# torognes/swarm

Hardware: AMD Instinct MI355X
Metric: amplicons/sec clustered (d=1) (higher is better)
Workload: dtype u64; 1 GPU; 10000000 synthetic amplicons x 150 bp, d=1 (10000000 per GPU; the metric's own size; configs[1]: configs1); per_gpu_queries=10000000, db_amplicons=10000000, step=swa_d1_index_build + swa_d1_network_device (B1 seam), db and CSR resident in HBM, route=streaming (d1_stream.inc), build=local, neighbour_links=17077441

## Files before the change

### swarm_amd/csrc/d1.hip

```cpp
#include "swa_internal.h"

#include <algorithm>
#include <type_traits>
#include <cstdlib>
#include <memory>
#include <thread>

namespace {

constexpr int kWaves = 4;
constexpr int kThreads = kWaves * 64;
constexpr int kQueueCap = 128;
constexpr size_t kMaxZobristLds = SWA_MAX_ZOBRIST_LDS;

#include "wave_ops.inc"
#include "group_join.inc"

struct alignas(16) swa_task {
  uint64_t hash;
  uint32_t heavy;
  uint32_t code;
};

struct NetArgs {
// ... 717 lines not shown
static int launch_abundance_rank(swa_ctx * ctx) {
  if (ctx->up.d1.rank_ready) {
    if (ctx->up.d1.db_unordered) { SWA_HIP(ctx, hipMemsetAsync(swa_status(ctx)->flags + kFlagUnordered, 1, sizeof(uint32_t), ctx->stream)); }
    return SWA_OK;
  }
  ctx->up.d1.rank_ready = true;
  SWA_HIP(ctx, hipMemsetAsync(swa_status(ctx)->flags + kFlagUnordered, 0, sizeof(uint32_t), ctx->stream));
  const uint32_t n = ctx->db.n;
  const uint32_t tiles = (n + 255u) / 256u;
  SWA_TRY(swa_reserve(ctx, ctx->d_arank, uint64_t(n) * sizeof(uint32_t)));
  SWA_TRY(swa_reserve(ctx, ctx->d_rank_tmp, uint64_t(tiles) * sizeof(uint32_t)));
  auto * rank = static_cast<uint32_t *>(ctx->d_arank.ptr);
  auto * tile_last = static_cast<uint32_t *>(ctx->d_rank_tmp.ptr);
  hipLaunchKernelGGL(k_abundance_rank, dim3(grid_for(ctx, n, 256, 8)), dim3(256), 0, ctx->stream, ctx->db.abundance, n, rank,
                     swa_status(ctx)->flags, tile_last);
  hipLaunchKernelGGL(k_abundance_rank_carry, dim3(1), dim3(256), 0, ctx->stream, tile_last, tiles);
  hipLaunchKernelGGL(k_abundance_rank_fill, dim3(grid_for(ctx, n, 256, 8)), dim3(256), 0, ctx->stream, n, rank, tile_last);
  return SWA_OK;
}

__global__ void k_set_flags(uint32_t * flags, uint32_t unserved, uint32_t shortest_code) { flags[kFlagUnserved] = unserved; flags[kFlagShortest] = shortest_code; }
__global__ void k_set_guard_made(unsigned long long * guard, uint32_t made0, uint32_t made1) { guard[kGuardMade] = made0; guard[kGuardMade + 1] = made1; }


using PartPlan = swa_part_levels;

struct PartJob {
  uint32_t nidx = 1;
  const unsigned long long * in[kMaxIdx] = {};
  unsigned long long * buf[kMaxIdx][2] = {};
  const uint64_t * cstart0[kMaxIdx] = {};
  uint64_t cstride0[kMaxIdx] = {};
  const uint32_t * csize0[kMaxIdx] = {};
  uint32_t csize_cap = 0, chunks0 = 1;
  bool single0 = true;
  uint64_t max_records = 0, max_tiles0 = 0;
  uint64_t out_cap = 0;
  uint32_t bias = 0, top_bit = 32;
  uint32_t tile = 4096;
  bool hist0_done = false;
  bool tiles0_done = false;
  const SegArgs * seg = nullptr;
  PartPlan plan{};
  uint32_t * cnt[kMaxIdx] = {}; uint32_t * ctile[kMaxIdx] = {}; uint64_t * starts[kMaxIdx] = {}; uint32_t * partial[kMaxIdx] = {};
  uint32_t * total[kMaxIdx] = {};
  uint64_t starts_stride = 0;
  const unsigned long long * out[kMaxIdx] = {}; const uint64_t * bstart[kMaxIdx] = {};
  uint32_t buckets = 0;
  int last = 0;
};

static void part_scratch(const PartJob & j, uint64_t * cnt, uint64_t * ctile, uint64_t * starts_half, uint64_t * partial) {
  uint64_t chunks = j.chunks0, c_max = 0, t_max = 0, s_max = 0;
  bool single = j.single0;
  for (uint32_t l = 0; l < j.plan.levels; ++l) {
    const uint64_t tiles = (l == 0 ? j.max_tiles0 : j.max_records / j.tile + chunks + 1);
    c_max = std::max(c_max, (tiles << j.plan.bits[l]) + 2);
    t_max = std::max(t_max, chunks + 2 + tiles + 2);
    chunks = (single ? 1 : chunks) << j.plan.bits[l];
    single = false;
    s_max = std::max(s_max, chunks + 2);
  }
  *cnt = c_max; *ctile = t_max; *starts_half = s_max; *partial = c_max / kFlatChunk + 2;
}

struct ClearList { uint32_t * p[8]; uint64_t words[8]; uint32_t n; };
__global__ __launch_bounds__(256) void k_clear_many(const ClearList c) {
  for (uint32_t k = 0; k < c.n; ++k) {
    for (uint64_t i = (uint64_t)blockIdx.x * blockDim.x + threadIdx.x; i < c.words[k]; i += (uint64_t)gridDim.x * blockDim.x) { c.p[k][i] = 0u; }
  }
}
static void clear_add(ClearList & c, void * p, uint64_t bytes) {
  c.p[c.n] = static_cast<uint32_t *>(p); c.words[c.n] = bytes / 4; ++c.n;
}
static int clear_launch(swa_ctx * ctx, const ClearList & c) {
  uint64_t most = 0;
  for (uint32_t k = 0; k < c.n; ++k) { most = std::max(most, c.words[k]); }
  if (c.n == 0 || most == 0) { return SWA_OK; }
  hipLaunchKernelGGL(k_clear_many, dim3(grid_for(ctx, most, 256, 8)), dim3(256), 0, ctx->stream, c);
  SWA_HIP(ctx, hipGetLastError());
  return SWA_OK;
}

static int run_partition(swa_ctx * ctx, PartJob & j) {
  uint64_t chunks = j.chunks0;
  bool single = j.single0;
  uint32_t used_bits = 0;
  const int cu_grid = ctx->num_cus * 8;
  for (uint32_t l = 0; l < j.plan.levels; ++l) {
    const uint32_t bits = j.plan.bits[l];
    used_bits += bits;
    const bool wide = bits > kPartMaxBits;
    const bool hist_done = l == 0 && j.hist0_done;
    const bool have_form = wide ? j.tile == 4096 || (j.tile == 8192 && hist_done) : j.tile == 2048 || j.tile == 4096;
    if (!have_form) { return swa_fail_msg(ctx, SWA_E_ARG, "partition: no kernel for this tile and bin count"); }
    PartArgs a{};
    a.single_seg = single ? 1u : 0u; a.bits = bits; a.shift = j.top_bit - used_bits; a.bias = j.bias; a.tile = j.tile;
    a.span = (single && l == 0 && chunks > 1 && j.tile == 4096 && !wide && !hist_done) ? 1u : 0u;
    const uint64_t tiles = (l == 0 ? j.max_tiles0 : j.max_records / j.tile + chunks + 1);
    a.run_bits = tiles >= (uint64_t)cu_grid ? 4u : 0u;
    for (uint32_t i = 0; i < j.nidx; ++i) {
      PartIdx & p = a.p[i];
      p.in = l == 0 ? j.in[i] : j.buf[i][(l - 1) & 1u];
      p.out = j.buf[i][l & 1u];
      p.out_cap = j.out_cap;
      p.cstart = l == 0 ? j.cstart0[i] : j.starts[i] + ((l - 1) & 1u) * j.starts_stride;
      p.cstride = l == 0 ? j.cstride0[i] : 0;
      p.csize = l == 0 ? j.csize0[i] : nullptr;
      p.csize_cap = j.csize_cap;
      p.chunks = (uint32_t)chunks;
      p.ctile = j.ctile[i]; p.cnt = j.cnt[i];
      p.tchunk = j.ctile[i] + chunks + 1; p.tchunk_cap = (uint32_t)std::min<uint64_t>(tiles + 1, 0xFFFFFFFFu);
      p.next_start = j.starts[i] + (l & 1u) * j.starts_stride;
      p.total = j.total[i];
    }
    const dim3 grid_t((unsigned)((std::min<uint64_t>(std::max<uint64_t>(tiles, 1), (uint64_t)cu_grid) + 7) & ~7ull), j.nidx);
    if (hist_done && j.tiles0_done) {  }
    else if (l == 0 && j.seg != nullptr) {
      if (chunks > 2048) { hipLaunchKernelGGL((k_part_tiles<1024, true>), dim3(1, 1), dim3(1024), 0, ctx->stream, a, *j.seg); }
      else { hipLaunchKernelGGL((k_part_tiles<256, true>), dim3(1, 1), dim3(256), 0, ctx->stream, a, *j.seg); }
    }
    else if (chunks > 2048) { hipLaunchKernelGGL(k_part_tiles<1024>, dim3(1, j.nidx), dim3(1024), 0, ctx->stream, a, SegArgs{}); }
    else { hipLaunchKernelGGL(k_part_tiles<256>, dim3(1, j.nidx), dim3(256), 0, ctx->stream, a, SegArgs{}); }
    if (hist_done) {  }
    else if (wide) { hipLaunchKernelGGL((k_part_hist<1024, kPartTileMax, 256>), grid_t, dim3(256), 0, ctx->stream, a); }
    else if (a.span != 0u) { hipLaunchKernelGGL((k_part_hist<512, kPartTileMax, 256, true>), grid_t, dim3(256), 0, ctx->stream, a); }
    else { hipLaunchKernelGGL((k_part_hist<512, kPartTileMax, 256>), grid_t, dim3(256), 0, ctx->stream, a); }
    FlatScanArgs f{};
    f.unit_bits = bits;
    for (uint32_t i = 0; i < j.nidx; ++i) { f.v[i] = j.cnt[i]; f.units[i] = j.ctile[i] + chunks; f.partial[i] = j.partial[i]; f.total[i] = j.total[i]; }
    const dim3 grid_f((unsigned)std::min<uint64_t>(((tiles << bits) + 1 + kFlatChunk - 1) / kFlatChunk, (uint64_t)cu_grid), j.nidx);
    hipLaunchKernelGGL(k_flat_sums, grid_f, dim3(256), 0, ctx->stream, f);
    hipLaunchKernelGGL(k_flat_apply, grid_f, dim3(256), 0, ctx->stream, f);
    if (wide && j.tile == 8192) {
      constexpr size_t lds = part_scatter_lds(8192, 1024);
      if (!ctx->part_lds_opt_in) {
        SWA_HIP(ctx, hipFuncSetAttribute(reinterpret_cast<const void *>(&k_part_scatter<8192, 1024, 1024>), hipFuncAttributeMaxDynamicSharedMemorySize, (int)lds));
        ctx->part_lds_opt_in = true;
      }
      hipLaunchKernelGGL((k_part_scatter<8192, 1024, 1024>), grid_t, dim3(1024), lds, ctx->stream, a);
    }
    else if (wide) { hipLaunchKernelGGL((k_part_scatter<4096, 1024, 512>), grid_t, dim3(512), part_scatter_lds(4096, 1024), ctx->stream, a); }
    else if (j.tile == 2048) { hipLaunchKernelGGL((k_part_scatter<2048, 512, 512>), grid_t, dim3(512), part_scatter_lds(2048, 512), ctx->stream, a); }
    else if (a.span != 0u) { hipLaunchKernelGGL((k_part_scatter<4096, 512, 512, true>), grid_t, dim3(512), part_scatter_lds(4096, 512), ctx->stream, a); }
    else { hipLaunchKernelGGL((k_part_scatter<4096, 512, 512>), grid_t, dim3(512), part_scatter_lds(4096, 512), ctx->stream, a); }
    chunks = (single ? 1 : chunks) << bits;
    single = false;
    SWA_HIP(ctx, hipGetLastError());
  }
  j.buckets = (uint32_t)chunks;
  j.last = (int)((j.plan.levels - 1) & 1u);
  for (uint32_t i = 0; i < j.nidx; ++i) {
    j.out[i] = j.buf[i][j.last];
    j.bstart[i] = j.starts[i] + (uint64_t)j.last * j.starts_stride;
  }
  return SWA_OK;
}

static int ensure_lines(swa_ctx * ctx) {
  const uint32_t lq = line_quads_for(ctx);
  if (ctx->up.d1.lines_ready && ctx->up.d1.lines_quads == lq) { return SWA_OK; }
  const uint32_t n = ctx->db.n;
  SWA_TRY(swa_reserve(ctx, ctx->d_stream[kSbLines], (uint64_t)n * lq * 16u + 64u));
  auto * lines = static_cast<uint4 *>(ctx->d_stream[kSbLines].ptr);
  const auto * rank = static_cast<const uint32_t *>(ctx->d_arank.ptr);
  SWA_HIP(ctx, hipMemsetAsync(reinterpret_cast<uint8_t *>(lines) + (uint64_t)n * lq * 16u, 0, 64, ctx->stream));
  swa_t0(ctx, kTimeLines);
  const dim3 grid(grid_for(ctx, n, 256, 8));
  if (lq == 4u) { hipLaunchKernelGGL(k_lines_build<4>, grid, dim3(256), 0, ctx->stream, ctx->db.seqs, ctx->db.seq_off, ctx->db.seqlen, rank, n, lines); }
  else if (lq == 8u) { hipLaunchKernelGGL(k_lines_build<8>, grid, dim3(256), 0, ctx->stream, ctx->db.seqs, ctx->db.seq_off, ctx->db.seqlen, rank, n, lines); }
  else { hipLaunchKernelGGL(k_lines_build<16>, grid, dim3(256), 0, ctx->stream, ctx->db.seqs, ctx->db.seq_off, ctx->db.seqlen, rank, n, lines); }
  swa_t1(ctx, kTimeLines);
  SWA_HIP(ctx, hipGetLastError());
  ctx->up.d1.lines_ready = true;
  ctx->up.d1.lines_quads = lq;
  return SWA_OK;
}

struct RouteLists {
  const uint32_t * ids[2] = {nullptr, nullptr};
  const unsigned long long * rec[2] = {nullptr, nullptr};
  uint32_t m[2] = {0, 0};
  bool routed() const { return ids[0] != nullptr || rec[0] != nullptr; }
  bool by_rec() const { return rec[0] != nullptr; }
};

static int build_stream_index(swa_ctx * ctx, const RouteLists & route) {
  const bool clear_head = ctx->ix.head_clear_pending;
  ctx->ix.head_clear_pending = false;
  ctx->ix.anchor_ready = false;
  ctx->ix.stream_index = false;
  ctx->ix.list_counts_ready = false;
  const uint32_t n = ctx->db.n;
  swa_status_block * st = swa_status(ctx);
  swa_lap(ctx, "(build starts)");
  SWA_TRY(ensure_db_lengths(ctx));
  swa_lap(ctx, "db lengths");
  SWA_TRY(ensure_lines(ctx));
  swa_lap(ctx, "amplicon lines");
  const uint32_t lq = ctx->up.d1.lines_quads;
  uint64_t item_room = 0;
  const ListRegions regions = list_regions(ctx, &item_room);
  const bool by_rec = route.by_rec();
  const bool routed = route.routed();
  const uint64_t records = routed ? std::max<uint64_t>(std::max(route.m[0], route.m[1]), 1) : n;
  uint32_t forced_bits = 0;
  if (const char * e = getenv("SWA_D1_PART_BITS")) {
    const int b = atoi(e);
    if (b >= 1 && b <= (int)(3 * kPartMaxBits)) { forced_bits = (uint32_t)b; }
  }
  const swa_part_plan plan = swa_part_plan_for(records, ctx->up.d1.stream_extra_bits, routed, forced_bits);
  const uint32_t total_bits = plan.lv.total;
  const bool keys_hist = plan.keys_hist;
  PartJob j;
  j.nidx = 2;
  j.plan = plan.lv;
  j.max_records = records;
  j.out_cap = records + 1;
  j.tile = plan.tile;
  swa_part_plan_report(plan, ctx->ix.part_plan);
  ctx->ix.part_plan[7] = ctx->up.d1.stream_extra_bits;
  ctx->ix.part_starts_valid = false;
  j.max_tiles0 = records / j.tile + 2;
// ... 59 lines not shown
    hipLaunchKernelGGL(k_set_flags, dim3(1), dim3(1), 0, ctx->stream, dflags,
                       ctx->up.d1.db_shortest < minlen ? 1u : 0u, 0xFFFFFFFFu - ctx->up.d1.db_shortest);
  }
  if (by_rec) {
    hipLaunchKernelGGL(k_set_guard_made, dim3(1), dim3(1), 0, ctx->stream, k.guard, route.m[0], route.m[1]);
  }
  swa_t0(ctx, kTimeKeys);
  if (by_rec) {  }
  else if (keys_hist) {
    const uint32_t ntiles = (uint32_t)((records + j.tile - 1) / j.tile);
    for (int i = 0; i < 2; ++i) {
      k.hist_cnt[i] = static_cast<uint32_t *>(ctx->d_stream[kSbCnt + i].ptr);
      k.hist_ctile[i] = static_cast<uint32_t *>(ctx->d_stream[kSbTile + i].ptr);
    }
    k.hist_bits = j.plan.bits[0]; k.hist_tile = j.tile; k.hist_ntiles = ntiles;
    k.hist_run_bits = j.max_tiles0 >= (uint64_t)ctx->num_cus * 8 ? 4u : 0u;
    const dim3 hgrid((unsigned)((std::min<uint64_t>(ntiles, (uint64_t)ctx->num_cus * 8) + 7) & ~7ull), 1u);
    hipLaunchKernelGGL(k_keys<true>, hgrid, dim3(256), 0, ctx->stream, k);
    j.hist0_done = true;
    j.tiles0_done = true;
  } else {
    const dim3 kgrid((unsigned)grid_for(ctx, records, 256, 8), routed ? 2u : 1u);
    hipLaunchKernelGGL(k_keys<false>, kgrid, dim3(256), 0, ctx->stream, k);
  }
  swa_t1(ctx, kTimeKeys);
  swa_lap(ctx, "k_keys");

  for (int i = 0; i < 2; ++i) {
    j.buf[i][0] = static_cast<unsigned long long *>(ctx->d_stream[kSbRec + 2 * i].ptr);
    j.buf[i][1] = static_cast<unsigned long long *>(ctx->d_stream[kSbRec + 2 * i + 1].ptr);
    j.in[i] = by_rec ? route.rec[i] : j.buf[i][1];
    j.cstart0[i] = nullptr; j.cstride0[i] = routed ? route.m[i] : n;
    j.cnt[i] = static_cast<uint32_t *>(ctx->d_stream[kSbCnt + i].ptr);
    j.ctile[i] = static_cast<uint32_t *>(ctx->d_stream[kSbTile + i].ptr);
    j.starts[i] = static_cast<uint64_t *>(ctx->d_stream[kSbStart + i].ptr);
    j.partial[i] = static_cast<uint32_t *>(ctx->d_stream[kSbPartial + i].ptr);
    j.total[i] = reinterpret_cast<uint32_t *>(scal + 8 + i);
  }
  j.starts_stride = e_start + 2;
  swa_t0(ctx, kTimeKeyPartition);
  SWA_TRY(run_partition(ctx, j));
  swa_t1(ctx, kTimeKeyPartition);
  swa_lap(ctx, "key partition");
  ctx->ix.part_starts_at = (uint64_t)(j.bstart[0] - j.starts[0]);
  ctx->ix.part_buckets = j.buckets;
  ctx->ix.part_starts_valid = true;
  if (!ctx->up.d1.guard_keys_done) {
    auto * guard = reinterpret_cast<unsigned long long *>(st->guard);
    SWA_HIP(ctx, hipMemsetAsync(guard + kGuardKeys, 0, sizeof(st->guard) - kGuardKeys * sizeof(uint64_t), ctx->stream));
    GuardDbArgs gd{};
    gd.seqs = ctx->db.seqs; gd.seq_off = ctx->db.seq_off; gd.seqlen = ctx->db.seqlen; gd.n = n;
    for (int i = 0; i < 2; ++i) { gd.list[i] = k.list[i]; gd.list_count[i] = routed ? route.m[i] : 0; gd.list_rec[i] = by_rec ? route.rec[i] : nullptr; }
    gd.owner_rank = k.owner_rank; gd.owner_world = k.owner_world; gd.win_a = win_a; gd.win_b = win_b; gd.nwin = k.nwin;
    gd.out = guard + kGuardKeysDb;
    hipLaunchKernelGGL(k_guard_db, dim3((unsigned)grid_for(ctx, records, 256, 8), routed ? 2u : 1u), dim3(256), 0, ctx->stream, gd);
    GuardRecArgs gr{};
    for (int i = 0; i < 2; ++i) { gr.rec[i] = j.out[i]; gr.total[i] = j.total[i]; }
    gr.out = guard + kGuardKeysRec;
    hipLaunchKernelGGL(k_guard_records, dim3((unsigned)grid_for(ctx, records, 256, 8), 2u), dim3(256), 0, ctx->stream, gr);
    ctx->up.d1.guard_keys_pending = true;
  }

  swa_lap(ctx, "guard: second opinion");
  GroupArgs g{};
  for (int i = 0; i < 2; ++i) {
    GroupIdx & x = g.g[i];
    x.rec = const_cast<unsigned long long *>(j.out[i]);
    x.bstart = j.bstart[i];
    x.buckets = j.buckets;
    x.members = static_cast<uint32_t *>(ctx->d_stream[kSbMembers + i].ptr);
    x.items_tmp = j.buf[i][j.last ^ 1];
    x.kind_cnt = static_cast<uint32_t *>(ctx->d_stream[kSbKind + i].ptr);
  }
  g.pair_big = kPairBigCap; g.group_cap = kStreamGroupCap;
  g.flags = dflags;
  g.guard = k.guard;
  g.over = static_cast<uint8_t *>(ctx->d_stream[kSbOver].ptr);
  swa_t0(ctx, kTimeGroups);
  {
    if (!ctx->g1_lds_opt_in) {
      SWA_HIP(ctx, hipFuncSetAttribute(reinterpret_cast<const void *>(&k_group1), hipFuncAttributeMaxDynamicSharedMemorySize, (int)kG1LdsBytes));
      ctx->g1_lds_opt_in = true;
    }
    hipLaunchKernelGGL(k_group1, dim3((unsigned)std::min<uint64_t>(buckets, (uint64_t)ctx->num_cus), 2), dim3(kG1Threads), kG1LdsBytes, ctx->stream, g);
  }
  swa_t1(ctx, kTimeGroups);

  FlatScanArgs f{};
  ListArgs la{};
  for (int i = 0; i < 2; ++i) {
    f.v[i] = g.g[i].kind_cnt; f.units[i] = nullptr; f.fixed[i] = (uint64_t)kListsPerIndex * buckets + 1;
    f.partial[i] = j.partial[i]; f.total[i] = reinterpret_cast<uint32_t *>(scal + 10 + i);
    ListIdx & x = la.x[i];
    x.items_tmp = g.g[i].items_tmp; x.bstart = g.g[i].bstart; x.kind_pos = g.g[i].kind_cnt; x.buckets = (uint32_t)buckets;
    x.l.items = static_cast<swa_item *>(ctx->d_aitems[i].ptr);
    x.l.region = regions;
    x.l.counters = st->counters + kCounterBase + (uint32_t)i * kWidthClasses * 8u;
    x.l.pair_big = g.pair_big;
  }
  const dim3 grid_l((unsigned)std::min<uint64_t>((buckets + 3) / 4, (uint64_t)ctx->num_cus * 8), 2);
  if (plan.lists_inline) {
    uint32_t mask = 0;
    for (uint32_t c = 0; c < kWidthClasses; ++c) { if (ctx->up.d1.class_pop[c] != 0) { mask |= ((1u << kListKinds) - 1u) << (c * kListKinds); } }
    for (int i = 0; i < 2; ++i) { la.x[i].list_mask = mask; }
    hipLaunchKernelGGL(k_group_lists<true>, grid_l, dim3(256), 0, ctx->stream, la);
  } else {
    const dim3 grid_k((unsigned)std::min<uint64_t>(((uint64_t)kListsPerIndex * buckets + kFlatChunk) / kFlatChunk, (uint64_t)ctx->num_cus * 8), 2);
    hipLaunchKernelGGL(k_flat_sums, grid_k, dim3(256), 0, ctx->stream, f);
    hipLaunchKernelGGL(k_flat_apply, grid_k, dim3(256), 0, ctx->stream, f);
    hipLaunchKernelGGL(k_group_lists<false>, grid_l, dim3(256), 0, ctx->stream, la);
  }
  ctx->ix.lists_form = plan.lists_inline ? 1 : 0;
  SWA_HIP(ctx, hipGetLastError());
  swa_lap(ctx, "groups + work lists");
  ctx->ix.list_regions_items = item_room;
  ctx->ix.anchor_ready = true;
  ctx->ix.stream_index = true;
  ctx->ix.guard_index = true;
  return SWA_OK;
}

static uint64_t csr_heavy_bytes(uint32_t count) { return ((1ull << swa_csr_plan_for(count).lv.total) + 2) * sizeof(uint32_t); }

static int csr_from_chunks(swa_ctx * ctx, uint32_t first, uint32_t count, const unsigned long long * links, const uint64_t * d_cstart, uint64_t cstride,
                           const uint32_t * d_csize, uint32_t chunks, uint32_t csize_cap, uint64_t max_tiles0, uint64_t link_cap,
                           uint64_t * d_offsets, uint32_t * d_neighbours, uint64_t cap, const SegArgs * seg = nullptr, bool heavy_cleared = false) {
  const swa_csr_plan plan = swa_csr_plan_for(count);
  const uint32_t nbits = plan.nbits, r = plan.r;
  PartJob j;
  j.nidx = 1;
  j.plan = plan.lv;
  j.max_records = link_cap;
  j.out_cap = link_cap;
  j.tile = 4096;
  j.max_tiles0 = max_tiles0;
  j.chunks0 = chunks; j.single0 = true; j.top_bit = nbits; j.bias = first;
  j.csize_cap = csize_cap;
  uint64_t e_cnt, e_tile, e_start, e_partial;
  part_scratch(j, &e_cnt, &e_tile, &e_start, &e_partial);
  SWA_TRY(swa_reserve(ctx, ctx->d_stream[kSbLinkA], (link_cap + 1) * sizeof(uint64_t)));
  SWA_TRY(swa_reserve(ctx, ctx->d_stream[kSbLinkB], (link_cap + 1) * sizeof(uint64_t)));
  SWA_TRY(swa_reserve(ctx, ctx->d_stream[kSbCnt], e_cnt * sizeof(uint32_t)));
  SWA_TRY(swa_reserve(ctx, ctx->d_stream[kSbTile], e_tile * sizeof(uint32_t)));
  SWA_TRY(swa_reserve(ctx, ctx->d_stream[kSbStart], (2 * e_start + 4) * sizeof(uint64_t)));
  SWA_TRY(swa_reserve(ctx, ctx->d_stream[kSbPartial], e_partial * sizeof(uint32_t)));
  SWA_TRY(swa_reserve(ctx, ctx->d_stream[kSbScal], 64 * sizeof(uint64_t)));
  j.in[0] = links;
  j.buf[0][0] = static_cast<unsigned long long *>(ctx->d_stream[kSbLinkA].ptr);
  j.buf[0][1] = static_cast<unsigned long long *>(ctx->d_stream[kSbLinkB].ptr);
  j.cstart0[0] = d_cstart; j.cstride0[0] = cstride;
  j.csize0[0] = d_csize;
  j.seg = d_csize != nullptr && j.nidx == 1 ? seg : nullptr;
  j.cnt[0] = static_cast<uint32_t *>(ctx->d_stream[kSbCnt].ptr);
  j.ctile[0] = static_cast<uint32_t *>(ctx->d_stream[kSbTile].ptr);
  j.starts[0] = static_cast<uint64_t *>(ctx->d_stream[kSbStart].ptr);
  ctx->ix.part_starts_valid = false;
  j.partial[0] = static_cast<uint32_t *>(ctx->d_stream[kSbPartial].ptr);
  j.total[0] = &swa_status(ctx)->links_sorted;
  j.starts_stride = e_start + 2;
  swa_t0(ctx, kTimeLinkPartition);
  SWA_TRY(run_partition(ctx, j));
  swa_t1(ctx, kTimeLinkPartition);
  CsrArgs c{};
  c.links = j.out[0]; c.bstart = j.bstart[0]; c.buckets = j.buckets; c.r = r; c.first = first; c.count = count;
  c.offsets = d_offsets; c.neighbours = d_neighbours; c.cap = d_neighbours != nullptr ? cap : 0;
  const void * heavy_before = ctx->d_stream[kSbHeavy].ptr;
  SWA_TRY(swa_reserve(ctx, ctx->d_stream[kSbHeavy], csr_heavy_bytes(count)));
// ... 1351 lines not shown
```

### swarm_amd/csrc/d1_stream.inc

```

constexpr uint32_t kPartTileMax = 4096;
constexpr uint32_t kPartMaxBits = SWA_PART_MAX_BITS;
constexpr unsigned long long kRecAbsent = ~0ull;
constexpr uint32_t kMaxIdx = 2;
constexpr uint32_t kStreamGroupCap = 4096;

template <int LQ>
__global__ __launch_bounds__(256) void k_lines_build(const uint64_t * __restrict__ seqs, const uint64_t * __restrict__ seq_off,
                                                     const uint32_t * __restrict__ seqlen, const uint32_t * __restrict__ rank, uint32_t n,
                                                     uint4 * __restrict__ lines) {
  constexpr uint32_t C = 2u * LQ - 1u;
  for (uint32_t i = blockIdx.x * blockDim.x + threadIdx.x; i < n; i += gridDim.x * blockDim.x) {
    const uint32_t len = seqlen[i];
    const uint64_t * s = seqs + seq_off[i];
    const uint32_t nw = (len + 31u) >> 5;
    uint32_t d[4 * LQ];
    d[0] = len; d[1] = rank[i];
#pragma unroll
    for (uint32_t k = 0; k < C; ++k) {
      const uint64_t w = k < nw ? s[k] : 0ull;
      d[2 + 2 * k] = (uint32_t)w; d[3 + 2 * k] = (uint32_t)(w >> 32);
    }
#pragma unroll
    for (uint32_t q = 0; q < (uint32_t)LQ; ++q) { lines[(uint64_t)i * LQ + q] = make_uint4(d[4 * q], d[4 * q + 1], d[4 * q + 2], d[4 * q + 3]); }
// ... 568 lines not shown
    }
    __syncthreads();
    for (uint32_t b = threadIdx.x; b < bins; b += THREADS) { p.cnt[part_flat(a, p, tile.c, t, b)] = hist[b]; }
    __syncthreads();
  }
}

constexpr uint32_t kFlatChunk = 4096;
constexpr uint32_t kFlatPer = kFlatChunk / 256u;
struct FlatScanArgs { uint32_t * v[kMaxIdx]; const uint32_t * units[kMaxIdx]; uint32_t unit_bits; uint64_t fixed[kMaxIdx]; uint32_t * partial[kMaxIdx]; uint32_t * total[kMaxIdx]; };
__device__ __forceinline__ uint64_t flat_length(const FlatScanArgs & a, uint32_t i) {
  return a.units[i] != nullptr ? ((uint64_t)*a.units[i] << a.unit_bits) + 1u : a.fixed[i];
}

__global__ __launch_bounds__(256) void k_flat_sums(const FlatScanArgs a) {
  __shared__ uint64_t smem[4];
  const uint32_t * v = a.v[blockIdx.y];
  const uint64_t m = flat_length(a, blockIdx.y);
  for (uint64_t blk = blockIdx.x; blk * kFlatChunk < m; blk += gridDim.x) {
    const uint64_t base = blk * kFlatChunk + (uint64_t)threadIdx.x * kFlatPer;
    uint64_t s = 0;
#pragma unroll
    for (uint32_t k = 0; k < kFlatPer; ++k) { if (base + k < m) { s += v[base + k]; } }
    uint64_t total;
    (void)block_exclusive_scan(s, smem, total);
    if (threadIdx.x == 0) { a.partial[blockIdx.y][blk] = (uint32_t)total; }
  }
}

__global__ __launch_bounds__(256) void k_flat_apply(const FlatScanArgs a) {
  __shared__ uint64_t smem[4];
  uint32_t * v = a.v[blockIdx.y];
  const uint64_t m = flat_length(a, blockIdx.y);
  const uint32_t * partial = a.partial[blockIdx.y];
  const uint64_t nblk = (m + kFlatChunk - 1) / kFlatChunk;
  for (uint64_t blk = blockIdx.x; blk < nblk; blk += gridDim.x) {
    uint64_t before = 0;
    for (uint64_t q = threadIdx.x; q < blk; q += 256u) { before += partial[q]; }
    uint64_t prefix;
    (void)block_exclusive_scan(before, smem, prefix);
    const uint64_t base = blk * kFlatChunk + (uint64_t)threadIdx.x * kFlatPer;
    uint32_t c[kFlatPer];
    uint64_t s = 0;
#pragma unroll
    for (uint32_t k = 0; k < kFlatPer; ++k) { c[k] = base + k < m ? v[base + k] : 0u; s += c[k]; }
    uint64_t total;
    uint64_t run = prefix + block_exclusive_scan(s, smem, total);
#pragma unroll
    for (uint32_t k = 0; k < kFlatPer; ++k) { if (base + k < m) { v[base + k] = (uint32_t)run; } run += c[k]; }
    if (blk + 1 == nblk && threadIdx.x == 0) { *a.total[blockIdx.y] = (uint32_t)(prefix + total); }
  }
}

template <uint32_t THREADS>
__device__ __forceinline__ uint64_t block_exclusive_scan_of(uint64_t v, uint64_t * smem, uint64_t & total) {
  const uint32_t lane = threadIdx.x & 63u, wave = threadIdx.x >> 6;
  uint64_t incl = v;
#pragma unroll
  for (unsigned d = 1; d < 64; d <<= 1) { const uint64_t t = swa_shfl_up_u64(incl, d); if (lane >= d) { incl += t; } }
  if (lane == 63u) { smem[wave] = incl; }
  __syncthreads();
  uint64_t wave_off = 0, tot = 0;
#pragma unroll
  for (uint32_t w = 0; w < THREADS / 64u; ++w) { const uint64_t x = smem[w]; wave_off += w < wave ? x : 0ull; tot += x; }
  __syncthreads();
  total = tot;
  return wave_off + incl - v;
}

__device__ __forceinline__ void part_write_starts(const PartArgs & a, const PartIdx & p) {
  const uint32_t buckets = (a.single_seg != 0u ? 1u : p.chunks) << a.bits;
  for (uint32_t i = blockIdx.x * blockDim.x + threadIdx.x; i <= buckets; i += gridDim.x * blockDim.x) {
    uint64_t at;
    if (i == buckets) { at = *p.total; }
    else if (a.single_seg != 0u) { at = p.cnt[(uint64_t)i * p.ctile[p.chunks]]; }
    else {
      const uint32_t c = i >> a.bits, b = i & ((1u << a.bits) - 1u), t0 = p.ctile[c];
      at = p.cnt[((uint64_t)t0 << a.bits) + (uint64_t)b * (p.ctile[c + 1] - t0)];
    }
    p.next_start[i] = at;
  }
}

template <uint32_t TILE, uint32_t BINS, uint32_t THREADS, bool SPAN = false>
__global__ __launch_bounds__(THREADS) __attribute__((amdgpu_waves_per_eu(SPAN && THREADS == 512 ? 8 : 1))) void k_part_scatter(const PartArgs a) {
  constexpr uint32_t kPartPer = TILE / THREADS;
  extern __shared__ __attribute__((aligned(16))) unsigned long long part_lds[];
  unsigned long long * stage = part_lds;
  uint32_t * hist = reinterpret_cast<uint32_t *>(stage + TILE);
  uint32_t * lstart = hist + BINS;
  uint32_t * goff = lstart + BINS;
  __shared__ uint64_t smem[THREADS / 64u];
  __shared__ uint32_t sh[1];
  __shared__ typename std::conditional<SPAN, SpanLds, uint32_t>::type span;
  const PartIdx & p = a.p[blockIdx.y];
  const uint32_t bins = 1u << a.bits;
  const uint32_t ntiles = p.ctile[p.chunks];
  for (uint32_t v = blockIdx.x; v < ((ntiles + (8u << a.run_bits) - 1u) & ~((8u << a.run_bits) - 1u)); v += gridDim.x) {
    const uint32_t t = xcd_tile(v, a.run_bits);
    if (t >= ntiles) { continue; }
    for (uint32_t b = threadIdx.x; b < bins; b += THREADS) { hist[b] = 0u; }
    PartTile tile{0u, 0u, 0ull};
    unsigned long long rec[kPartPer];
    uint32_t pos[kPartPer];
    const auto digit_of = [&](unsigned long long r) { return (((uint32_t)(r >> 32) - a.bias) >> a.shift) & (bins - 1u); };
    if constexpr (SPAN) {
#pragma unroll
      for (uint32_t k = 0; k < kPartPer; ++k) { rec[k] = kRecAbsent; pos[k] = 0u; }
      (void)part_span<kPartPer, THREADS>(p, TILE, t, span, [&](uint32_t k, uint64_t place) {
        rec[k] = p.in[place];
        if (rec[k] != kRecAbsent) { pos[k] = atomicAdd(&hist[digit_of(rec[k])], 1u); }
      });
    } else {
      tile = part_tile(p, TILE, t, sh);
#pragma unroll
      for (uint32_t k = 0; k < kPartPer; ++k) {
        const uint32_t j = k * THREADS + threadIdx.x;
        rec[k] = kRecAbsent; pos[k] = 0u;
        if (j < tile.count) { rec[k] = p.in[tile.first + j]; }
        if (rec[k] != kRecAbsent) { pos[k] = atomicAdd(&hist[digit_of(rec[k])], 1u); }
      }
    }
    __syncthreads();
    {
      constexpr uint32_t kB = (BINS + THREADS - 1u) / THREADS;
      uint32_t h[kB];
      uint64_t sum = 0;
#pragma unroll
      for (uint32_t q = 0; q < kB; ++q) { const uint32_t b = kB * threadIdx.x + q; h[q] = b < bins ? hist[b] : 0u; sum += h[q]; }
      uint64_t total;
      uint32_t run = (uint32_t)block_exclusive_scan_of<THREADS>(sum, smem, total);
#pragma unroll
      for (uint32_t q = 0; q < kB; ++q) {
        const uint32_t b = kB * threadIdx.x + q;
        if (b < bins) { lstart[b] = run; goff[b] = p.cnt[part_flat(a, p, tile.c, t, b)]; }
        run += h[q];
      }
    }
    __syncthreads();
#pragma unroll
    for (uint32_t k = 0; k < kPartPer; ++k) {
      if (rec[k] != kRecAbsent) {
        const uint32_t at = lstart[(((uint32_t)(rec[k] >> 32) - a.bias) >> a.shift) & (bins - 1u)] + pos[k];
        stage[at] = rec[k];
      }
    }
    __syncthreads();
    const uint32_t present = lstart[bins - 1u] + hist[bins - 1u];
#pragma unroll
    for (uint32_t k = 0; k < kPartPer; ++k) {
      const uint32_t j = k * THREADS + threadIdx.x;
      if (j < present) {
        const unsigned long long r = stage[j];
        const uint32_t d = (((uint32_t)(r >> 32) - a.bias) >> a.shift) & (bins - 1u);
        const uint64_t g = (uint64_t)goff[d] + (j - lstart[d]);
        if (g < p.out_cap) {
          p.out[g] = r;
        }
      }
    }
    __syncthreads();
  }
  part_write_starts(a, p);
}

constexpr size_t part_scatter_lds(uint32_t tile, uint32_t bins) { return (size_t)tile * 8u + 3u * (size_t)bins * 4u; }

struct GroupIdx {
  unsigned long long * rec;
  const uint64_t * bstart;
  uint32_t buckets;
  uint32_t * members;
  unsigned long long * items_tmp;
  uint32_t * kind_cnt;
};
struct GroupArgs {
  GroupIdx g[kMaxIdx];
  uint32_t pair_big, group_cap;
  uint32_t * flags;
  unsigned long long * guard;
// ... 702 lines not shown
```

Before: 6.143 billion amplicons/s.

## Pipeline next-tile loads in wide 8192-tile partition scatter with smaller persistent grid

```diff
diff --git a/swarm_amd/csrc/d1.hip b/swarm_amd/csrc/d1.hip
--- a/swarm_amd/csrc/d1.hip
+++ b/swarm_amd/csrc/d1.hip
@@ -823,11 +823,20 @@
   return SWA_OK;
 }
 
+static uint32_t stream_grid_hook() {
+  if (const char * e = getenv("SWA_D1_STREAM_GRID")) {
+    const int v = atoi(e);
+    if (v >= 1 && v <= 65535) { return (uint32_t)v; }
+  }
+  return 0u;
+}
+
 static int run_partition(swa_ctx * ctx, PartJob & j) {
   uint64_t chunks = j.chunks0;
   bool single = j.single0;
   uint32_t used_bits = 0;
-  const int cu_grid = ctx->num_cus * 8;
+  const uint32_t hook_grid = stream_grid_hook();
+  const int cu_grid = hook_grid != 0u ? (int)((hook_grid + 7u) & ~7u) : ctx->num_cus * 8;
   for (uint32_t l = 0; l < j.plan.levels; ++l) {
     const uint32_t bits = j.plan.bits[l];
     used_bits += bits;
@@ -839,7 +848,9 @@
     a.single_seg = single ? 1u : 0u; a.bits = bits; a.shift = j.top_bit - used_bits; a.bias = j.bias; a.tile = j.tile;
     a.span = (single && l == 0 && chunks > 1 && j.tile == 4096 && !wide && !hist_done) ? 1u : 0u;
     const uint64_t tiles = (l == 0 ? j.max_tiles0 : j.max_records / j.tile + chunks + 1);
-    a.run_bits = tiles >= (uint64_t)cu_grid ? 4u : 0u;
+    const bool pipe = wide && j.tile == 8192;
+    const int in_flight = !pipe || hook_grid != 0u ? cu_grid : std::max(8, (ctx->num_cus / (int)std::max(1u, j.nidx)) & ~7);
+    a.run_bits = tiles >= (uint64_t)in_flight ? 4u : 0u;
     for (uint32_t i = 0; i < j.nidx; ++i) {
       PartIdx & p = a.p[i];
       p.in = l == 0 ? j.in[i] : j.buf[i][(l - 1) & 1u];
@@ -855,7 +866,7 @@
       p.next_start = j.starts[i] + (l & 1u) * j.starts_stride;
       p.total = j.total[i];
     }
-    const dim3 grid_t((unsigned)((std::min<uint64_t>(std::max<uint64_t>(tiles, 1), (uint64_t)cu_grid) + 7) & ~7ull), j.nidx);
+    const dim3 grid_t((unsigned)((std::min<uint64_t>(std::max<uint64_t>(tiles, 1), (uint64_t)in_flight) + 7) & ~7ull), j.nidx);
     if (hist_done && j.tiles0_done) {  }
     else if (l == 0 && j.seg != nullptr) {
       if (chunks > 2048) { hipLaunchKernelGGL((k_part_tiles<1024, true>), dim3(1, 1), dim3(1024), 0, ctx->stream, a, *j.seg); }
@@ -876,10 +887,10 @@
     if (wide && j.tile == 8192) {
       constexpr size_t lds = part_scatter_lds(8192, 1024);
       if (!ctx->part_lds_opt_in) {
-        SWA_HIP(ctx, hipFuncSetAttribute(reinterpret_cast<const void *>(&k_part_scatter<8192, 1024, 1024>), hipFuncAttributeMaxDynamicSharedMemorySize, (int)lds));
+        SWA_HIP(ctx, hipFuncSetAttribute(reinterpret_cast<const void *>(&k_part_scatter<8192, 1024, 1024, false, true>), hipFuncAttributeMaxDynamicSharedMemorySize, (int)lds));
         ctx->part_lds_opt_in = true;
       }
-      hipLaunchKernelGGL((k_part_scatter<8192, 1024, 1024>), grid_t, dim3(1024), lds, ctx->stream, a);
+      hipLaunchKernelGGL((k_part_scatter<8192, 1024, 1024, false, true>), grid_t, dim3(1024), lds, ctx->stream, a);
     }
     else if (wide) { hipLaunchKernelGGL((k_part_scatter<4096, 1024, 512>), grid_t, dim3(512), part_scatter_lds(4096, 1024), ctx->stream, a); }
     else if (j.tile == 2048) { hipLaunchKernelGGL((k_part_scatter<2048, 512, 512>), grid_t, dim3(512), part_scatter_lds(2048, 512), ctx->stream, a); }
@@ -1105,7 +1116,8 @@
       SWA_HIP(ctx, hipFuncSetAttribute(reinterpret_cast<const void *>(&k_group1), hipFuncAttributeMaxDynamicSharedMemorySize, (int)kG1LdsBytes));
       ctx->g1_lds_opt_in = true;
     }
-    hipLaunchKernelGGL(k_group1, dim3((unsigned)std::min<uint64_t>(buckets, (uint64_t)ctx->num_cus), 2), dim3(kG1Threads), kG1LdsBytes, ctx->stream, g);
+    const uint32_t hook_grid = stream_grid_hook();
+    hipLaunchKernelGGL(k_group1, dim3((unsigned)std::min<uint64_t>(buckets, hook_grid != 0u ? (uint64_t)hook_grid : (uint64_t)ctx->num_cus), 2), dim3(kG1Threads), kG1LdsBytes, ctx->stream, g);
   }
   swa_t1(ctx, kTimeGroups);
 
diff --git a/swarm_amd/csrc/d1_stream.inc b/swarm_amd/csrc/d1_stream.inc
--- a/swarm_amd/csrc/d1_stream.inc
+++ b/swarm_amd/csrc/d1_stream.inc
@@ -674,7 +674,7 @@
   }
 }
 
-template <uint32_t TILE, uint32_t BINS, uint32_t THREADS, bool SPAN = false>
+template <uint32_t TILE, uint32_t BINS, uint32_t THREADS, bool SPAN = false, bool PIPE = false>
 __global__ __launch_bounds__(THREADS) __attribute__((amdgpu_waves_per_eu(SPAN && THREADS == 512 ? 8 : 1))) void k_part_scatter(const PartArgs a) {
   constexpr uint32_t kPartPer = TILE / THREADS;
   extern __shared__ __attribute__((aligned(16))) unsigned long long part_lds[];
@@ -688,6 +688,94 @@
   const PartIdx & p = a.p[blockIdx.y];
   const uint32_t bins = 1u << a.bits;
   const uint32_t ntiles = p.ctile[p.chunks];
+  if constexpr (PIPE) {
+    static_assert(!SPAN, "the pipelined walk cuts its tiles chunk by chunk");
+    constexpr uint32_t kB = (BINS + THREADS - 1u) / THREADS;
+    const uint32_t vend = (ntiles + (8u << a.run_bits) - 1u) & ~((8u << a.run_bits) - 1u);
+    const auto turn_from = [&](uint32_t v) {
+      while (v < vend && xcd_tile(v, a.run_bits) >= ntiles) { v += gridDim.x; }
+      return v;
+    };
+    unsigned long long rec[kPartPer];
+    uint32_t gpre[kB];
+    const auto ask = [&](uint32_t t, uint32_t c) {
+      const uint32_t within = (t - p.ctile[c]) * TILE;
+      const uint64_t first = part_chunk_base(p, c) + within;
+      const uint32_t count = min(TILE, part_chunk_size(p, c) - within);
+#pragma unroll
+      for (uint32_t k = 0; k < kPartPer; ++k) {
+        const uint32_t j = k * THREADS + threadIdx.x;
+        rec[k] = j < count ? p.in[first + j] : kRecAbsent;
+      }
+#pragma unroll
+      for (uint32_t q = 0; q < kB; ++q) {
+        const uint32_t b = kB * threadIdx.x + q;
+        gpre[q] = b < bins ? p.cnt[part_flat(a, p, c, t, b)] : 0u;
+      }
+    };
+    uint32_t v = turn_from(blockIdx.x);
+    if (v < vend) {
+      if (threadIdx.x == 0) { sh[0] = part_chunk_of(p.ctile, p.chunks, xcd_tile(v, a.run_bits)); }
+      __syncthreads();
+      ask(xcd_tile(v, a.run_bits), sh[0]);
+      __syncthreads();
+    }
+    while (v < vend) {
+      const uint32_t vn = turn_from(v + gridDim.x);
+      const uint32_t tn = vn < vend ? xcd_tile(vn, a.run_bits) : 0u;
+      for (uint32_t b = threadIdx.x; b < bins; b += THREADS) { hist[b] = 0u; }
+      if (vn < vend && threadIdx.x == 0) { sh[0] = part_chunk_of(p.ctile, p.chunks, tn); }
+      __syncthreads();
+      uint32_t pos[kPartPer];
+#pragma unroll
+      for (uint32_t k = 0; k < kPartPer; ++k) {
+        pos[k] = 0u;
+        if (rec[k] != kRecAbsent) { pos[k] = atomicAdd(&hist[(((uint32_t)(rec[k] >> 32) - a.bias) >> a.shift) & (bins - 1u)], 1u); }
+      }
+      __syncthreads();
+      {
+        uint32_t h[kB];
+        uint64_t sum = 0;
+#pragma unroll
+        for (uint32_t q = 0; q < kB; ++q) { const uint32_t b = kB * threadIdx.x + q; h[q] = b < bins ? hist[b] : 0u; sum += h[q]; }
+        uint64_t total;
+        uint32_t run = (uint32_t)block_exclusive_scan_of<THREADS>(sum, smem, total);
+#pragma unroll
+        for (uint32_t q = 0; q < kB; ++q) {
+          const uint32_t b = kB * threadIdx.x + q;
+          if (b < bins) { lstart[b] = run; goff[b] = gpre[q]; }
+          run += h[q];
+        }
+      }
+      __syncthreads();
+#pragma unroll
+      for (uint32_t k = 0; k < kPartPer; ++k) {
+        if (rec[k] != kRecAbsent) {
+          const uint32_t at = lstart[(((uint32_t)(rec[k] >> 32) - a.bias) >> a.shift) & (bins - 1u)] + pos[k];
+          stage[at] = rec[k];
+        }
+      }
+      __syncthreads();
+      const uint32_t present = lstart[bins - 1u] + hist[bins - 1u];
+      if (vn < vend) { ask(tn, sh[0]); }
+#pragma unroll
+      for (uint32_t k = 0; k < kPartPer; ++k) {
+        const uint32_t j = k * THREADS + threadIdx.x;
+        if (j < present) {
+          const unsigned long long r = stage[j];
+          const uint32_t d = (((uint32_t)(r >> 32) - a.bias) >> a.shift) & (bins - 1u);
+          const uint64_t g = (uint64_t)goff[d] + (j - lstart[d]);
+          if (g < p.out_cap) {
+            p.out[g] = r;
+          }
+        }
+      }
+      __syncthreads();
+      v = vn;
+    }
+    part_write_starts(a, p);
+    return;
+  }
   for (uint32_t v = blockIdx.x; v < ((ntiles + (8u << a.run_bits) - 1u) & ~((8u << a.run_bits) - 1u)); v += gridDim.x) {
     const uint32_t t = xcd_tile(v, a.run_bits);
     if (t >= ntiles) { continue; }
```

Result: faster. 6.269 billion amplicons/s, median of 6 (+2.0%).
